# CDACHPCIE25/PPQSFLHE

Hardware: AMD Instinct MI355X
Metric: ciphertexts/sec aggregated+PRE at N=2^16, L=12 RNS limbs (higher is better)
Workload: dtype u64

## Files before the change

### ppqsflhe_amd/csrc/engine.hip

```cpp
#include "engine.hpp"
#include "comm.hpp"
#include "ntt_radix.hpp"
#include "qsum_kernels.hpp"
#include "fanout_kernels.hpp"
#include "codec_kernels.hpp"
#include "sampler_kernels.hpp"

#include <cmath>
#include <cstdio>
#include <type_traits>
#include <cstdlib>
#include <cstring>

namespace mk {


template <bool INV>
__global__ __launch_bounds__(NTT_THREADS) void k_ntt_col(NttIo io, NttTables T, const u64 *scale,
                                                         const u64 *scale_sh) {
    extern __shared__ __attribute__((aligned(16))) u64 lds[];
    const uint32_t poly = blockIdx.y / io.nslots, s = blockIdx.y % io.nslots;
    if (ntt_slot_skipped(io, poly, io.vslot0 + s)) return;
    const uint32_t id = limb_id_of(io.vslot0 + s, io.nl, T.L);
    const LimbConst lc = T.limb[id];
// ... 361 lines not shown

static int fast_row(uint32_t log_r2, uint32_t rows);

static dim3 ew_grid(uint32_t n, uint32_t slots, uint32_t items) {
    return dim3((n / 2 + EW_THREADS - 1) / EW_THREADS, slots, items);
}

static std::string hip_runtime_diagnosis() {
    std::vector<std::string> paths;
    if (FILE *f = std::fopen("/proc/self/maps", "r")) {
        char line[4096];
        while (std::fgets(line, sizeof line, f)) {
            const char *p = std::strstr(line, "libamdhip64");
            if (!p) continue;
            const char *start = std::strchr(line, '/');
            if (!start) continue;
            std::string path(start);
            while (!path.empty() && (path.back() == '\n' || path.back() == ' ')) path.pop_back();
            bool seen = false;
            for (const std::string &q : paths) seen = seen || q == path;
            if (!seen) paths.push_back(path);
        }
        std::fclose(f);
    }
    if (paths.size() < 2) return "";
    std::string msg = "; this process carries " + std::to_string(paths.size()) + " HIP runtimes (";
    for (size_t i = 0; i < paths.size(); ++i) msg += (i ? ", " : "") + paths[i];
    return msg + "): the one initialised second sees no device -- load the library that owns the device first (import torch "
                 "before libmkckks_hip.so, or link both against the same libamdhip64)";
}

static bool env_flag(const char *name, bool dflt) {
    const char *e = std::getenv(name);
    return e ? std::atoi(e) != 0 : dflt;
}
Knobs Knobs::from_env() {
    Knobs k;
    if (const char *e = std::getenv("MKCKKS_CHUNK")) {
        const int v = std::atoi(e);
        if (v >= 1 && v <= 64) k.chunk = (uint32_t)v;
    }
    if (const char *e = std::getenv("MKCKKS_QSUM_GROUP")) {
        const int v = std::atoi(e);
        if (v >= 1 && v <= 64) k.qsum_group = (uint32_t)v;
    }
    if (const char *e = std::getenv("MKCKKS_FANOUT_GROUP")) {
        const int v = std::atoi(e);
        if (v >= 1 && v <= 64) k.fanout_group = (uint32_t)v;
    }
    k.cu_affine = env_flag("MKCKKS_CU_AFFINE", k.cu_affine);
    k.generic_ntt = env_flag("MKCKKS_GENERIC_NTT", k.generic_ntt);
    k.no_pm = env_flag("MKCKKS_NO_PM", k.no_pm);
    k.no_fp64 = env_flag("MKCKKS_NO_FP64", k.no_fp64);
    return k;
}

Engine::Engine(const ParamSet &ps, int device) : ps_(ps), device_(device), knobs_(Knobs::from_env()) {
    if (device_ < 0) return;
    int count = 0;
    if (hipGetDeviceCount(&count) != hipSuccess || count <= device_)
        throw NoDevice("no HIP device " + std::to_string(device_) + " (found " + std::to_string(count) + ")" +
                       hip_runtime_diagnosis());
    MK_HIP(hipSetDevice(device_));
    const uint32_t D = ps_.D, n = ps_.n;
    tabs_.log_n = ps_.log_n;
    tabs_.log_r1 = (ps_.log_n % 2 == 0) ? ((ps_.log_n / 2) & ~1u) : ps_.log_n / 2;
    tabs_.log_r2 = ps_.log_n - tabs_.log_r1;
    if (knobs_.generic_ntt) { tabs_.log_r1 = ps_.log_n / 2; tabs_.log_r2 = ps_.log_n - tabs_.log_r1; }
    const bool radix_both = fast_log_h(tabs_.log_r1, 1u << tabs_.log_r2) && fast_row(tabs_.log_r2, 1u << tabs_.log_r1);
    const bool fp_ok = radix_both && !knobs_.no_fp64;
    tabs_.has_fp = 0;
    fp_of_.assign(D, 0);
    for (uint32_t i = 0; i < D; ++i) {
        ps_.limb[i].fp = (fp_ok && ps_.moduli[i] < (5ull << 48)) ? 1u : 0u;
        fp_of_[i] = (uint8_t)ps_.limb[i].fp;
        tabs_.has_fp |= ps_.limb[i].fp;
    }
    bool all_pm = radix_both && !knobs_.no_pm;
    for (uint32_t i = 0; i < D; ++i)
        if (!ps_.limb[i].fp && !pm_eligible(ps_.moduli[i])) all_pm = false;
    tabs_.int_pm = all_pm ? 1u : 0u;
    for (uint32_t i = 0; i < D; ++i) {
        const bool pm = all_pm && !ps_.limb[i].fp;
        ps_.limb[i].pm = pm ? 1u : 0u;
        ps_.limb[i].pm_c = pm ? (uint32_t)(((u64)1 << ps_.limb[i].k) - ps_.moduli[i]) : 0u;
    }
    tabs_.h_fp_of = fp_of_.data();
    tabs_.cu_affine = knobs_.cu_affine ? 1u : 0u;
    tabs_.stamps = nullptr;
    if (MK_STAMP && env_flag("MKCKKS_STAMPS", false)) {
        MK_HIP(hipMalloc(&d_stamps_, (size_t)STAMP_REGIONS * STAMP_REGION * sizeof(unsigned long long)));
        MK_HIP(hipMemset(d_stamps_, 0, (size_t)STAMP_REGIONS * STAMP_REGION * sizeof(unsigned long long)));
        tabs_.stamps = d_stamps_;
    }
    MK_HIP(hipMalloc(&d_limb_, D * sizeof(LimbConst)));
    MK_HIP(hipMemcpy(d_limb_, ps_.limb.data(), D * sizeof(LimbConst), hipMemcpyHostToDevice));
    const size_t tbytes = (size_t)D * n * sizeof(u64);
    MK_HIP(hipMalloc(&d_tw_, tbytes));
    MK_HIP(hipMalloc(&d_tw_sh_, tbytes));
    MK_HIP(hipMalloc(&d_itw_, tbytes));
    MK_HIP(hipMalloc(&d_itw_sh_, tbytes));
    std::vector<u64> w, wsh;
    auto as_fp = [&](uint32_t i) {
        const long double q = (long double)ps_.moduli[i];
        for (uint32_t k = 0; k < n; ++k) {
            const double wd = (double)w[k], wq = (double)((long double)w[k] / q);
            std::memcpy(&w[k], &wd, 8);
            std::memcpy(&wsh[k], &wq, 8);
        }
    };
    auto as_pm = [&](uint32_t i) {
        for (uint32_t k = 0; k < n; ++k) {
            wsh[k] = pm_tw_companion(w[k], ps_.limb[i]);
            w[k] = pm_tw(w[k], ps_.limb[i]);
        }
    };
    for (uint32_t i = 0; i < D; ++i) {
        ps_.twiddles(i, false, w, wsh);
        if (ps_.limb[i].fp) as_fp(i);
        if (ps_.limb[i].pm) as_pm(i);
        MK_HIP(hipMemcpy(d_tw_ + (size_t)i * n, w.data(), n * sizeof(u64), hipMemcpyHostToDevice));
        MK_HIP(hipMemcpy(d_tw_sh_ + (size_t)i * n, wsh.data(), n * sizeof(u64), hipMemcpyHostToDevice));
        ps_.twiddles(i, true, w, wsh);
        if (ps_.limb[i].fp) as_fp(i);
        if (ps_.limb[i].pm) as_pm(i);
        MK_HIP(hipMemcpy(d_itw_ + (size_t)i * n, w.data(), n * sizeof(u64), hipMemcpyHostToDevice));
        MK_HIP(hipMemcpy(d_itw_sh_ + (size_t)i * n, wsh.data(), n * sizeof(u64), hipMemcpyHostToDevice));
    }
    {
        const uint32_t slots = n / 2, M = 2 * n;
        std::vector<uint32_t> rot(slots);
        uint64_t pw = 1;
        for (uint32_t j = 0; j < slots; ++j) { rot[j] = (uint32_t)pw; pw = pw * 5 % M; }
        std::vector<double2> ksi(M + 1);
        const double pi = std::acos(-1.0);
        for (uint32_t k = 0; k <= M; ++k) {
            const double ang = 2.0 * pi * (double)k / (double)M;
            ksi[k] = double2{std::cos(ang), std::sin(ang)};
        }
        MK_HIP(hipMalloc(&d_rot_, slots * sizeof(uint32_t)));
        MK_HIP(hipMalloc(&d_ksi_, (M + 1) * sizeof(double2)));
// ... 375 lines not shown
                [&](hipStream_t s) { k_ntt_row3<INV, AR_FP><<<dim3((r1 / 4) * itemsf), NTT_THREADS, 0, s>>>(iof, T, tail); });
            break;
        case 4:
            launch_two_classes(ln, items != 0, itemsf != 0,
                [&](hipStream_t s) { with_int_arith(T, [&](auto ar) {
                    k_ntt_row_r<4, INV, decltype(ar)::value>
                        <<<dim3((r1 / 16) * items), NTT_THREADS, 0, s>>>(io, T, tail);
                }); },
                [&](hipStream_t s) { k_ntt_row_r<4, INV, AR_FP><<<dim3((r1 / 16) * itemsf), NTT_THREADS, 0, s>>>(iof, T, tail); });
            break;
        case 3:
            launch_two_classes(ln, items != 0, itemsf != 0,
                [&](hipStream_t s) { with_int_arith(T, [&](auto ar) {
                    k_ntt_row_r<3, INV, decltype(ar)::value>
                        <<<dim3((r1 / 32) * items), NTT_THREADS, 0, s>>>(io, T, tail);
                }); },
                [&](hipStream_t s) { k_ntt_row_r<3, INV, AR_FP><<<dim3((r1 / 32) * itemsf), NTT_THREADS, 0, s>>>(iof, T, tail); });
            break;
        case 2:
            launch_two_classes(ln, items != 0, itemsf != 0,
                [&](hipStream_t s) { with_int_arith(T, [&](auto ar) {
                    k_ntt_row_r<2, INV, decltype(ar)::value>
                        <<<dim3((r1 / 64) * items), NTT_THREADS, 0, s>>>(io, T, tail);
                }); },
                [&](hipStream_t s) { k_ntt_row_r<2, INV, AR_FP><<<dim3((r1 / 64) * itemsf), NTT_THREADS, 0, s>>>(iof, T, tail); });
            break;
        default: {
            if (tail.enabled) throw std::logic_error("fused tail needs the radix row kernel");
            const uint32_t tile = n < (uint32_t)NTT_TILE ? n : (uint32_t)NTT_TILE;
            k_ntt_row<INV><<<dim3(n / tile, n_polys * io0.nslots), NTT_THREADS, (size_t)tile * sizeof(u64), ln.main>>>(io0, T);
        }
    }
}

static void ntt_passes(NttIo io, const NttTables &T, uint32_t n_polys, bool inverse, const u64 *scale,
                       const u64 *scale_sh, const Lanes &s, int pack = 0) {
    if (n_polys == 0 || io.nslots == 0) return;
    NttIo second = io;
    second.in_group = 0;
    second.in = io.out;
    second.in_stride = io.out_stride;
    second.in_slot0 = io.out_slot0;
    const TailArgs none{};
    if (!inverse) {
        launch_col<false>(io, T, n_polys, nullptr, nullptr, s);
        launch_row<false>(second, T, n_polys, none, s);
    } else {
        launch_row<true>(io, T, n_polys, none, s);
        launch_col<true>(second, T, n_polys, scale, scale_sh, s, pack);
    }
    MK_HIP(hipGetLastError());
}

template <int LOG_H, int N_IN, int SRCMODE>
static void launch_conv_col_n(const ConvIo &io, const ConvIo &iof, const dim3 &grid, const dim3 &gridf, const NttTables &T,
                              const DevConv &cv, const Lanes &ln) {
    if constexpr (LOG_H >= 3) {
        const uint32_t per = grid.x / (io.nsel ? io.nsel : 1), perf = gridf.x / (iof.nsel ? iof.nsel : 1);
        if (io.nsel) with_int_arith(T, [&](auto ar) {
            k_conv_col2<LOG_H, N_IN, decltype(ar)::value, DevConv, SRCMODE>
                <<<dim3(per * ((io.nsel + 1) / 2)), NTT_THREADS, 0, ln.main>>>(io, T, cv);
        });
        if (iof.nsel)
            k_conv_col2<LOG_H, N_IN, AR_FP, DevConv, SRCMODE><<<dim3(perf * ((iof.nsel + 1) / 2)), NTT_THREADS, 0, ln.main>>>(iof, T, cv);
    } else {
        launch_two_classes(ln, io.nsel != 0, iof.nsel != 0,
            [&](hipStream_t s) { with_int_arith(T, [&](auto ar) {
                k_conv_col<LOG_H, N_IN, decltype(ar)::value, DevConv, SRCMODE>
                    <<<grid, NTT_THREADS, 0, s>>>(io, T, cv);
            }); },
            [&](hipStream_t s) { k_conv_col<LOG_H, N_IN, AR_FP, DevConv, SRCMODE><<<gridf, NTT_THREADS, 0, s>>>(iof, T, cv); });
    }
}
template <int LOG_H, int N_IN>
static void launch_conv_col_m(const ConvIo &io, const ConvIo &iof, const dim3 &grid, const dim3 &gridf, const NttTables &T,
                              const DevConv &cv, const Lanes &ln, int srcmode) {
    if constexpr (N_IN <= 4 && LOG_H >= 3) {
        if (srcmode == 1) return launch_conv_col_n<LOG_H, N_IN, 1>(io, iof, grid, gridf, T, cv, ln);
        if (srcmode == 2) return launch_conv_col_n<LOG_H, N_IN, (N_IN > 1 ? 2 : 0)>(io, iof, grid, gridf, T, cv, ln);
    }
    if (srcmode != 0) throw std::logic_error("double conversion sources: unsupported shape");
    launch_conv_col_n<LOG_H, N_IN, 0>(io, iof, grid, gridf, T, cv, ln);
}
template <int LOG_H>
static void launch_conv_col_h(const ConvIo &io0, const NttTables &T, const DevConv &cv, const Lanes &ln, int srcmode,
                              unsigned classes) {
    const uint32_t tiles = (1u << T.log_r2) / (256u >> LOG_H);
    ConvIo io = io0, iof = io0;
    io.target_mask = iof.target_mask = 0;
    for (uint32_t j = 0; j < cv.n_out; ++j) {
        const bool fp = T.h_fp_of[cv.dst_id[j]] != 0;
        if (fp && (classes & 2)) iof.target_mask |= 1ull << j;
        if (!fp && (classes & 1)) io.target_mask |= 1ull << j;
    }
    io.nsel = (uint32_t)__builtin_popcountll(io.target_mask);
    iof.nsel = (uint32_t)__builtin_popcountll(iof.target_mask);
    const dim3 grid(io.items * tiles * io.nsel), gridf(io.items * tiles * iof.nsel);
    switch (cv.n_in) {
        case 1: launch_conv_col_m<LOG_H, 1>(io, iof, grid, gridf, T, cv, ln, srcmode); break;
        case 2: launch_conv_col_m<LOG_H, 2>(io, iof, grid, gridf, T, cv, ln, srcmode); break;
        case 3: launch_conv_col_m<LOG_H, 3>(io, iof, grid, gridf, T, cv, ln, srcmode); break;
        case 4: launch_conv_col_m<LOG_H, 4>(io, iof, grid, gridf, T, cv, ln, srcmode); break;
        case 5: launch_conv_col_m<LOG_H, 5>(io, iof, grid, gridf, T, cv, ln, srcmode); break;
        case 6: launch_conv_col_m<LOG_H, 6>(io, iof, grid, gridf, T, cv, ln, srcmode); break;
        case 7: launch_conv_col_m<LOG_H, 7>(io, iof, grid, gridf, T, cv, ln, srcmode); break;
        case 8: launch_conv_col_m<LOG_H, 8>(io, iof, grid, gridf, T, cv, ln, srcmode); break;
        default: throw std::invalid_argument("base conversion fan-in unsupported");
    }
}
// ... 1118 lines not shown
```

### ppqsflhe_amd/csrc/engine.hpp

```cpp
#pragma once
#include <hip/hip_runtime.h>

#include <map>
#include <stdexcept>
#include <string>
#include <utility>
#include <vector>

#include "modarith.hpp"
#include "ntt_kernels.hpp"
#include "params.hpp"

namespace mk {

struct HipError : std::runtime_error {
    using std::runtime_error::runtime_error;
};
struct NoDevice : std::runtime_error {
    using std::runtime_error::runtime_error;
};
struct PrecisionError : std::runtime_error {
    using std::runtime_error::runtime_error;
};

#define MK_HIP(expr)                                                                              \
    do {                                                                                          \
        hipError_t _e = (expr);                                                                   \
        if (_e != hipSuccess)                                                                     \
            throw mk::HipError(std::string(#expr) + ": " + hipGetErrorString(_e) + " (" __FILE__ \
                               ":" + std::to_string(__LINE__) + ")");                             \
    } while (0)

constexpr int MAX_CONV_IN = 8;
constexpr int MAX_CONV_OUT = 40;

struct DevConv {
    uint32_t n_in, n_out;
    uint32_t src_id[MAX_CONV_IN];
    uint32_t src_slot[MAX_CONV_IN];
    uint32_t dst_id[MAX_CONV_OUT];
    uint32_t dst_slot[MAX_CONV_OUT];
    u64 hatinv[MAX_CONV_IN], hatinv_sh[MAX_CONV_IN];
    const u64 *hat;
    const double *hat_d;
    const double *hatq_d;
};

struct Lanes {
    hipStream_t main = nullptr;
};

struct Knobs {
    uint32_t chunk = 16;
    uint32_t fanout_group = 7;
    uint32_t qsum_group = 8;
    bool cu_affine = true;
    bool generic_ntt = false;
    bool no_pm = false;
    bool no_fp64 = false;
    static Knobs from_env();
};

class Engine {
public:
    explicit Engine(const ParamSet &ps, int device);
    ~Engine();
    Engine(const Engine &) = delete;
    Engine &operator=(const Engine &) = delete;

    const ParamSet &params() const { return ps_; }
    bool has_device() const { return device_ >= 0; }
    int device() const { return device_; }
    void set_stream(hipStream_t s) { stream_ = s; }
    hipStream_t stream() const { return stream_; }
    void sync();

    void *dev_alloc(size_t bytes);
    void dev_free(void *p);
    void upload(void *d, const void *h, size_t bytes);
    void download(void *h, const void *d, size_t bytes);
    void *host_alloc(size_t bytes);
    void host_free(void *p);
    uint64_t upload_async(void *d, const void *h, size_t bytes);
    uint64_t download_async(void *h, const void *d, size_t bytes);
    bool copy_done(uint64_t ticket);
    void copy_wait(uint64_t ticket);
    void fence_uploads();
    void fence_compute();
    uint64_t count_noncanonical(const u64 *ct, uint32_t n_ct, uint32_t nl);

    void ntt_forward(u64 *d, uint32_t n_polys, uint32_t nl, bool with_p);
    void ntt_inverse(u64 *d, uint32_t n_polys, uint32_t nl, bool with_p);

    void eval_add(const u64 *a, const u64 *b, u64 *out, uint32_t n_ct, uint32_t nl);
    void eval_sum(const u64 *in, u64 *out, uint32_t n_clients, uint32_t n_ct, uint32_t nl);
    void rescale(const u64 *in, u64 *out, uint32_t n_ct, uint32_t nl, const std::vector<u64> *factors);
    void mult_const(u64 *ct, uint32_t n_ct, uint32_t nl, const std::vector<u64> &factors);
    void reduce_mod(u64 *ct, uint32_t n_ct, uint32_t nl, uint32_t n_terms);
    void reduce_scatter_sum_mod(void *comm, const u64 *partial, u64 *shard, uint32_t n_ct_shard, uint32_t nl,
                                uint32_t n_ranks);

    void reencrypt_sum(const u64 *cts, const u64 *evks, u64 *out, uint32_t n_clients, uint32_t n_ct, uint32_t nl);
    void reencrypt_fanout(const u64 *ct, const u64 *evks, u64 *out, uint32_t n_keys, uint32_t n_ct, uint32_t nl);
    void compress(const u64 *in, u64 *out, uint32_t n_ct, uint32_t nl_in, uint32_t nl_out);
    void reencrypt_fanout_compact(const u64 *ct, const u64 *evks, u64 *out, uint32_t n_keys, uint32_t n_ct, uint32_t nl_in,
                                  uint32_t nl_out);
    void modup(const u64 *c1, u64 *digits, uint32_t n, uint32_t nl);
    void moddown(const u64 *in, u64 *out, uint32_t n, uint32_t nl);
    void reencrypt(const u64 *ct, const u64 *evk, u64 *out, uint32_t n_ct, uint32_t nl, bool accumulate = false);

    void keygen(const int8_t *s, const u64 *a, const int32_t *e, u64 *pk, u64 *sk);
    void rekeygen(const int8_t *s_old, const u64 *pk_new, const int8_t *u, const int32_t *e0,
// ... 85 lines not shown
```

### ppqsflhe_amd/csrc/ntt_kernels.hpp

```cpp
#pragma once
#include "modarith.hpp"

namespace mk {

constexpr int NTT_THREADS = 256;
constexpr int NTT_TILE = 4096;
constexpr int NTT_COLS = 16;

struct NttTables {
    const LimbConst *limb;
    const u64 *tw, *tw_sh;
    const u64 *itw, *itw_sh;
    const u64 *twb, *itwb;
    uint32_t log_n, log_r1, log_r2;
    uint32_t L;
    uint32_t has_fp;
    const unsigned char *h_fp_of;
    uint32_t int_pm;
    unsigned long long *stamps;
    uint32_t cu_affine;
};
constexpr int AR_INT = 0, AR_FP = 1, AR_PM = 2;

struct NttIo {
    const u64 *in;
    u64 *out;
    size_t in_stride, out_stride;
    uint32_t in_slot0, out_slot0;
    uint32_t vslot0;
    uint32_t nslots;
    uint32_t nl;
    uint32_t skip_nparts = 0, skip_alpha = 0;
    unsigned long long slot_mask = ~0ull;
    uint32_t nsel = 0;
    uint32_t in_group = 0;
    size_t in_gstride = 0;
};
MK_D size_t ntt_in_offset(const NttIo &io, uint32_t poly) {
    return io.in_group ? (size_t)(poly / io.in_group) * io.in_gstride + (size_t)(poly % io.in_group) * io.in_stride
                       : (size_t)poly * io.in_stride;
}

MK_D uint32_t nth_set_bit(unsigned long long mask, uint32_t n) {
    for (uint32_t i = 0; i < n; ++i) mask &= mask - 1;
    return (uint32_t)__builtin_ctzll(mask);
}

MK_D bool ntt_slot_skipped(const NttIo &io, uint32_t poly, uint32_t vslot) {
    if (!io.skip_nparts) return false;
    const uint32_t lo = (poly % io.skip_nparts) * io.skip_alpha;
    const uint32_t hi = lo + io.skip_alpha < io.nl ? lo + io.skip_alpha : io.nl;
    return vslot >= lo && vslot < hi;
}

MK_D uint32_t limb_id_of(uint32_t vslot, uint32_t nl, uint32_t L) {
    return vslot < nl ? vslot : L + (vslot - nl);
}

MK_D void ct_butterfly(u64 &x, u64 &y, u64 w, u64 wp, u64 q, u64 q2) {
    u64 u = csub(x, q2);
    u64 v = shoup_lazy(y, w, wp, q);
    x = u + v;
    y = u - v + q2;
}
MK_D void ct_butterfly_c4(u64 &x, u64 &y, u64 w, u64 wp, u64 q, u64 q2, u64 q4) {
    u64 u = csub(x, q4);
    u64 v = shoup_lazy(y, w, wp, q);
    x = u + v;
    y = u - v + q2;
}
MK_D void ct_butterfly_nc(u64 &x, u64 &y, u64 w, u64 wp, u64 q, u64 q2) {
    u64 v = shoup_lazy(y, w, wp, q);
    u64 u = x;
// ... 68 lines not shown
```

### ppqsflhe_amd/csrc/ntt_radix.hpp

```cpp
#pragma once
#include "modarith.hpp"
#include "ntt_kernels.hpp"

namespace mk {

#ifndef MK_NT8
#define MK_NT8 0
#endif
MK_D u64 ld_stream(const u64 *p) { return (MK_NT && MK_NT8) ? __builtin_nontemporal_load(p) : *p; }
MK_D ulong2 ld_stream2(const ulong2 *p) {
    if (MK_NT) {
        ulong2 v;
        v.x = __builtin_nontemporal_load(&p->x);
        v.y = __builtin_nontemporal_load(&p->y);
        return v;
    }
    return *p;
}
MK_D u64 ld_pass(const u64 *p) { return (MK_NT >= 2 && MK_NT8) ? __builtin_nontemporal_load(p) : *p; }
#ifndef MK_NT8S
#define MK_NT8S 1
#endif
MK_D void st_pass(u64 *p, u64 v) {
    if (MK_NT >= 2 && MK_NT8S) __builtin_nontemporal_store(v, p);
// ... 514 lines not shown
#pragma unroll
            for (int k = 0; k < H; ++k) {
                const u64 v = (AR == AR_FP) ? fp_to_canonical(fp_mulmod(bitsd(x[k]), bitsd(sc), bitsd(sc_sh), lc.qd), lc.qd, lc.qinv)
                                 : shoup_mul(x[k], sc, sc_sh, lc.q);
                st_pass(dst + (size_t)(j + H * k) * r2, pack30(v));
            }
        } else {
#pragma unroll
            for (int k = 0; k < H; ++k) {
                const u64 v = (AR == AR_FP) ? fp_to_canonical(fp_mulmod(bitsd(x[k]), bitsd(sc), bitsd(sc_sh), lc.qd), lc.qd, lc.qinv)
                                 : shoup_mul(x[k], sc, sc_sh, lc.q);
                st_pass(dst + (size_t)(j + H * k) * r2, v);
            }
        }
    }
}

struct ConvIo {
    const u64 *in;
    u64 *out;
    size_t in_stride, out_stride;
    uint32_t items;
    unsigned long long target_mask;
    uint32_t nsel;
};
#ifndef MK_CONV_DEPTH
#define MK_CONV_DEPTH 6
#endif
#ifndef MK_PROBE
#define MK_PROBE 0
#endif
#if MK_PROBE == 1
#define MK_PROBE_SRC(src, limb_off, row_off) (src)[(limb_off) + (size_t)j * r2 + 0 * (row_off)]
#elif MK_PROBE == 2
#define MK_PROBE_SRC(src, limb_off, row_off) ((u64)threadIdx.x * 0x9E3779B97F4A7C15ull + (limb_off) + (row_off))
#else
#define MK_PROBE_SRC(src, limb_off, row_off) (src)[(limb_off) + (row_off)]
#endif

MK_D void split30_d(u64 dbl_bits, uint32_t &lo, uint32_t &hi) {
    const u64 b = dbits(bitsd(dbl_bits) + 4503599627370496.0) & 0xFFFFFFFFFFFFFull;
    lo = (uint32_t)b & 0x3FFFFFFFu;
    hi = (uint32_t)(b >> 30);
}
template <int SRCMODE>
MK_D constexpr bool src_is_double(int i) {
    return SRCMODE == 1 || (SRCMODE == 2 && i > 0);
}
template <int N_IN>
struct ConvConst {
    uint32_t h0[N_IN], h1[N_IN];
    double hd[N_IN], hq[N_IN];
};
template <int N_IN, int AR, int SRCMODE, typename CONV>
MK_D void conv_consts(const CONV &cv, uint32_t jt, ConvConst<N_IN> &k) {
#pragma unroll
    for (int i = 0; i < N_IN; ++i) {
        if ((AR == AR_FP) && src_is_double<SRCMODE>(i)) {
            k.hd[i] = cv.hat_d[i * cv.n_out + jt];
            k.hq[i] = cv.hatq_d[i * cv.n_out + jt];
        } else {
            split30(cv.hat[i * cv.n_out + jt], k.h0[i], k.h1[i]);
        }
    }
}
template <int N_IN, int SRCMODE>
MK_D void conv_split_sources(const u64 (&p)[N_IN], uint32_t (&a0)[N_IN], uint32_t (&a1)[N_IN]) {
#pragma unroll
    for (int i = 0; i < N_IN; ++i) {
        if (src_is_double<SRCMODE>(i)) {
            split30_d(p[i], a0[i], a1[i]);
        } else {
            a0[i] = (uint32_t)p[i];
            a1[i] = (uint32_t)(p[i] >> 32);
        }
    }
}
template <int N_IN, int AR, int SRCMODE>
MK_D u64 conv_output(const u64 (&p)[N_IN], const uint32_t (&a0)[N_IN], const uint32_t (&a1)[N_IN], const ConvConst<N_IN> &k,
                     const LimbConst &lc) {
    if ((AR == AR_FP) && SRCMODE != 0) {
        double acc = 0.0;
        if (SRCMODE == 2) {
            Cols ia{0, 0, 0};
#pragma unroll
            for (int i = 0; i < N_IN; ++i)
                if (!src_is_double<SRCMODE>(i)) mac_cols(ia, (uint32_t)p[i], (uint32_t)(p[i] >> 32), k.h0[i], k.h1[i]);
            acc = (double)reduce_cols_lazy(ia, lc);
        }
#pragma unroll
        for (int i = 0; i < N_IN; ++i)
            if (src_is_double<SRCMODE>(i)) acc += fp_mulmod(bitsd(p[i]), k.hd[i], k.hq[i], lc.qd);
        return dbits(fp_reduce(acc, lc.qd, lc.qinv));
    }
    Cols acc{0, 0, 0};
#pragma unroll
    for (int i = 0; i < N_IN; ++i) mac_cols(acc, a0[i], a1[i], k.h0[i], k.h1[i]);
    const u64 v = AR == AR_PM ? pm_reduce_cols(acc, pm_consts(lc)) : reduce_cols_lazy(acc, lc);
    return AR == AR_FP ? dbits(fp_reduce((double)v, lc.qd, lc.qinv)) : v;
}

template <int LOG_H, int N_IN, int AR, typename CONV, int SRCMODE = 0>
__global__ __launch_bounds__(NTT_THREADS, 4) void k_conv_col(ConvIo io, NttTables T, CONV cv) {
    using TL = ColTile<LOG_H>;
    constexpr int H = TL::H, S = TL::S;
    static_assert(SRCMODE == 0 || N_IN <= 4, "double sources: at most 4 per digit");
    __shared__ u64 lds[TL::WORDS + ColTwB<LOG_H>::WORDS];
    const uint32_t n = 1u << T.log_n, r2 = 1u << T.log_r2, tiles = r2 / S;
    const uint32_t groups = io.items * tiles;
    uint32_t grp, jt;
    group_member(blockIdx.x, groups, io.nsel, T.cu_affine, grp, jt);
    jt = nth_set_bit(io.target_mask, jt);
    uint32_t item, tile;
    conv_item_tile(grp, groups, io.items, tiles, item, tile);
    const uint32_t id = cv.dst_id[jt];
// ... 7 lines not shown
    stm.mark<0>();
    if constexpr (N_IN <= 4) {
        ConvConst<N_IN> kc;
        conv_consts<N_IN, AR, SRCMODE>(cv, jt, kc);
        constexpr int DEPTH = MK_CONV_DEPTH < H ? MK_CONV_DEPTH : H;
        u64 ring[DEPTH][N_IN];
#pragma unroll
        for (int k = 0; k < DEPTH; ++k)
#pragma unroll
            for (int i = 0; i < N_IN; ++i) ring[k][i] = MK_PROBE_SRC(src, (size_t)cv.src_slot[i] * n, (size_t)(j + H * k) * r2);
#pragma unroll
        for (int k = 0; k < H; ++k) {
            u64 p[N_IN];
#pragma unroll
            for (int i = 0; i < N_IN; ++i) p[i] = ring[k % DEPTH][i];
            if (k + DEPTH < H) {
#pragma unroll
                for (int i = 0; i < N_IN; ++i)
                    ring[k % DEPTH][i] = MK_PROBE_SRC(src, (size_t)cv.src_slot[i] * n, (size_t)(j + H * (k + DEPTH)) * r2);
            }
            uint32_t a0[N_IN], a1[N_IN];
            if (!((AR == AR_FP) && SRCMODE != 0)) conv_split_sources<N_IN, SRCMODE>(p, a0, a1);
            x[k] = conv_output<N_IN, AR, SRCMODE>(p, a0, a1, kc, lc);
            asm volatile("" : "+v"(x[k]));
            __builtin_amdgcn_sched_barrier(0);
        }
    } else {
        uint32_t h0[N_IN], h1[N_IN];
#pragma unroll
        for (int i = 0; i < N_IN; ++i) split30(cv.hat[i * cv.n_out + jt], h0[i], h1[i]);
#pragma unroll
        for (int k = 0; k < H; ++k) {
            Cols4 acc{0, 0, 0, 0};
#pragma unroll
            for (int i = 0; i < N_IN; ++i) {
                const u64 p = src[(size_t)cv.src_slot[i] * n + (size_t)(j + H * k) * r2];
                mac_cols4(acc, (uint32_t)p, (uint32_t)(p >> 32), h0[i], h1[i]);
            }
            x[k] = reduce_cols4(acc, lc);
            if (AR == AR_FP) x[k] = dbits(fp_reduce((double)x[k], lc.qd, lc.qinv));
            asm volatile("" : "+v"(x[k]));
            __builtin_amdgcn_sched_barrier(0);
        }
    }
    stm.mark<1>();
    col_forward_finish<LOG_H, AR>(x, lds, T.tw + (size_t)id * n, T.tw_sh + (size_t)id * n, lc, j, c, dst, r2, &stm);
    if (AR == AR_FP) stm.flush<0>(T.stamps, true);
    else stm.flush<1>(T.stamps, true);
}

#ifndef MK_CONV2_DEPTH
#define MK_CONV2_DEPTH 4
#endif
template <int LOG_H, int N_IN, int AR, typename CONV, int SRCMODE = 0>
__global__ __launch_bounds__(NTT_THREADS, 3) void k_conv_col2(ConvIo io, NttTables T, CONV cv) {
    using TL = ColTile<LOG_H>;
    constexpr int H = TL::H, S = TL::S;
    static_assert(SRCMODE == 0 || N_IN <= 4, "double sources: at most 4 per digit");
    __shared__ u64 lds[TL::WORDS + ColTwB<LOG_H>::WORDS];
    const uint32_t n = 1u << T.log_n, r2 = 1u << T.log_r2, tiles = r2 / S;
    const uint32_t groups = io.items * tiles, ntg = (io.nsel + 1) / 2;
    uint32_t grp, jg;
    group_member(blockIdx.x, groups, ntg, T.cu_affine, grp, jg);
    const bool two = jg * 2 + 1 < io.nsel;
    const uint32_t jta = nth_set_bit(io.target_mask, jg * 2), jtb = two ? nth_set_bit(io.target_mask, jg * 2 + 1) : jta;
    uint32_t item, tile;
    conv_item_tile(grp, groups, io.items, tiles, item, tile);
    const uint32_t ida = cv.dst_id[jta], idb = cv.dst_id[jtb];
    const LimbConst la = T.limb[ida], lb = T.limb[idb];
    if ((la.fp != 0) != (AR == AR_FP) || (lb.fp != 0) != (AR == AR_FP)) return;
    const int c = threadIdx.x % S, j = threadIdx.x / S;
    const u64 *src = io.in + (size_t)item * io.in_stride + tile * S + c;
    u64 xa[H], xb[H];
    if constexpr (N_IN > 4) {
        uint32_t h0a[N_IN], h1a[N_IN], h0b[N_IN], h1b[N_IN];
#pragma unroll
        for (int i = 0; i < N_IN; ++i) {
            split30(cv.hat[i * cv.n_out + jta], h0a[i], h1a[i]);
            split30(cv.hat[i * cv.n_out + jtb], h0b[i], h1b[i]);
        }
#pragma unroll
        for (int k = 0; k < H; ++k) {
            Cols4 acca{0, 0, 0, 0}, accb{0, 0, 0, 0};
#pragma unroll
            for (int i = 0; i < N_IN; ++i) {
                const u64 p = src[(size_t)cv.src_slot[i] * n + (size_t)(j + H * k) * r2];
                mac_cols4(acca, (uint32_t)p, (uint32_t)(p >> 32), h0a[i], h1a[i]);
                mac_cols4(accb, (uint32_t)p, (uint32_t)(p >> 32), h0b[i], h1b[i]);
            }
            xa[k] = reduce_cols4(acca, la);
            xb[k] = reduce_cols4(accb, lb);
            if (AR == AR_FP) {
                xa[k] = dbits(fp_reduce((double)xa[k], la.qd, la.qinv));
                xb[k] = dbits(fp_reduce((double)xb[k], lb.qd, lb.qinv));
            }
            asm volatile("" : "+v"(xa[k]), "+v"(xb[k]));
            __builtin_amdgcn_sched_barrier(0);
        }
    } else {
    ConvConst<N_IN> ka, kb;
    conv_consts<N_IN, AR, SRCMODE>(cv, jta, ka);
    conv_consts<N_IN, AR, SRCMODE>(cv, jtb, kb);
    constexpr int DEPTH = MK_CONV2_DEPTH < H ? MK_CONV2_DEPTH : H;
    u64 ring[DEPTH][N_IN];
#pragma unroll
    for (int k = 0; k < DEPTH; ++k)
#pragma unroll
        for (int i = 0; i < N_IN; ++i) ring[k][i] = src[(size_t)cv.src_slot[i] * n + (size_t)(j + H * k) * r2];
#pragma unroll
    for (int k = 0; k < H; ++k) {
        u64 p[N_IN];
#pragma unroll
        for (int i = 0; i < N_IN; ++i) p[i] = ring[k % DEPTH][i];
        if (k + DEPTH < H) {
#pragma unroll
            for (int i = 0; i < N_IN; ++i)
                ring[k % DEPTH][i] = src[(size_t)cv.src_slot[i] * n + (size_t)(j + H * (k + DEPTH)) * r2];
        }
        uint32_t a0[N_IN], a1[N_IN];
        if (!((AR == AR_FP) && SRCMODE != 0)) conv_split_sources<N_IN, SRCMODE>(p, a0, a1);
        xa[k] = conv_output<N_IN, AR, SRCMODE>(p, a0, a1, ka, la);
        xb[k] = conv_output<N_IN, AR, SRCMODE>(p, a0, a1, kb, lb);
        asm volatile("" : "+v"(xa[k]), "+v"(xb[k]));
        __builtin_amdgcn_sched_barrier(0);
    }
    }
    u64 *dst = io.out + (size_t)item * io.out_stride + (size_t)cv.dst_slot[jta] * n + tile * S + c;
    col_forward_finish<LOG_H, AR>(xa, lds, T.tw + (size_t)ida * n, T.tw_sh + (size_t)ida * n, la, j, c, dst, r2);
    if (!two) return;
    __syncthreads();
    dst = io.out + (size_t)item * io.out_stride + (size_t)cv.dst_slot[jtb] * n + tile * S + c;
    const u64 *twb = T.tw + (size_t)idb * n, *twb_sh = T.tw_sh + (size_t)idb * n;
    asm volatile("" : "+s"(twb), "+s"(twb_sh));
    col_forward_finish<LOG_H, AR>(xb, lds, twb, twb_sh, lb, j, c, dst, r2);
}

template <int LOG_H, int AR>
__global__ __launch_bounds__(NTT_THREADS, 3) void k_icol_sum(const u64 *pc, u64 *psum, NttTables T, const u64 *scale,
                                                             const u64 *scale_sh, uint32_t K, uint32_t n_clients,
                                                             size_t in_cstride) {
    using TL = ColTile<LOG_H>;
    constexpr int H = TL::H, S = TL::S;
    static_assert(AR != AR_FP, "P limbs are integer-class");
    __shared__ u64 lds[TL::WORDS + ColTwB<LOG_H>::WORDS];
    const uint32_t poly = blockIdx.y / K, k = blockIdx.y % K;
    const uint32_t id = T.L + k;
    const LimbConst lc = T.limb[id];
    const uint32_t n = 1u << T.log_n, r2 = 1u << T.log_r2;
    const int c = threadIdx.x % S, j = threadIdx.x / S;
    const size_t off = ((size_t)poly * K + k) * n + blockIdx.x * S + c;
    const u64 *itw0 = T.itw + (size_t)id * n, *itw_sh0 = T.itw_sh + (size_t)id * n;
    const u64 sc = scale[id], sc_sh = scale_sh[id];
    u64 acc[H];
#pragma unroll
    for (int kk = 0; kk < H; ++kk) acc[kk] = 0;
    ColTwB<LOG_H>::stage(lds + TL::WORDS, itw0, itw_sh0);
    wave_lds_sync();
    const u64 *strip = lds + TL::WORDS;
#pragma unroll 1
    for (uint32_t cl = 0; cl < n_clients; ++cl) {
        const u64 *src = pc + (size_t)cl * in_cstride + off;
        u64 x[H];
        uint32_t r2v = r2;
        asm volatile("" : "+s"(r2v));
#pragma unroll
        for (int kk = 0; kk < H; ++kk) x[kk] = ld_pass(src + (uint32_t)(H * j + kk) * r2v);
        radix_inverse_staged<LOG_H, AR>(x, [&](int i) { return ColTwB<LOG_H>::pair_b(strip, j, i); }, lc);
        if (cl) __syncthreads();
#pragma unroll
        for (int kk = 0; kk < H; ++kk) lds[TL::at(j, kk, c)] = x[kk];
        __syncthreads();
#pragma unroll
        for (int kk = 0; kk < H; ++kk) x[kk] = lds[TL::at(kk, j, c)];
        radix_inverse_staged<LOG_H, AR>(x, [&](int i) { return ColTwB<LOG_H>::pair_a(strip, i); }, lc);
#pragma unroll
        for (int kk = 0; kk < H; ++kk) acc[kk] += shoup_mul(x[kk], sc, sc_sh, lc.q);
    }
    u64 *dst = psum + off;
#pragma unroll
    for (int kk = 0; kk < H; ++kk) st_pass(dst + (size_t)(j + H * kk) * r2, acc[kk]);
}

template <int LOG_H, int N_IN, int AR, typename CONV>
__global__ __launch_bounds__(NTT_THREADS, 4) void k_conv_col_psum(ConvIo io, NttTables T, CONV cv) {
    using TL = ColTile<LOG_H>;
    constexpr int H = TL::H, S = TL::S;
    __shared__ u64 lds[TL::WORDS + ColTwB<LOG_H>::WORDS];
// ... 1059 lines not shown
```

Before: 31710.

## Merge int and fp basis-conversion column launches into one mixed-pair kernel

Adds a k_conv_col_mix kernel that handles integer-class and fp64-class conversion targets in a single launch. Targets are paired host-side, preferring same-class pairs and producing at most one mixed pair, and blocks are placed onto CUs with an optional two-CU grouping scheme. It also moves per-target hat constants into scalar registers via readfirstlane. The aim is to remove a separate launch, fill the GPU better, and lower VGPR pressure. The cost is extra template instantiations and branching, and the mixed pair may be unbalanced.

```diff
diff --git a/ppqsflhe_amd/csrc/engine.hip b/ppqsflhe_amd/csrc/engine.hip
--- a/ppqsflhe_amd/csrc/engine.hip
+++ b/ppqsflhe_amd/csrc/engine.hip
@@ -437,6 +437,10 @@
     k.generic_ntt = env_flag("MKCKKS_GENERIC_NTT", k.generic_ntt);
     k.no_pm = env_flag("MKCKKS_NO_PM", k.no_pm);
     k.no_fp64 = env_flag("MKCKKS_NO_FP64", k.no_fp64);
+    if (const char *e = std::getenv("MKCKKS_CONV_SPLIT")) {
+        const int v = std::atoi(e);
+        if (v >= 0 && v <= 3) k.conv_split = (uint32_t)v;
+    }
     return k;
 }
 
@@ -472,6 +476,7 @@
     }
     tabs_.h_fp_of = fp_of_.data();
     tabs_.cu_affine = knobs_.cu_affine ? 1u : 0u;
+    tabs_.conv_split = knobs_.conv_split;
     tabs_.stamps = nullptr;
     if (MK_STAMP && env_flag("MKCKKS_STAMPS", false)) {
         MK_HIP(hipMalloc(&d_stamps_, (size_t)STAMP_REGIONS * STAMP_REGION * sizeof(unsigned long long)));
@@ -953,9 +958,40 @@
     MK_HIP(hipGetLastError());
 }
 
+static ConvPairs conv_pairs(unsigned long long mask_int, unsigned long long mask_fp) {
+    static_assert(MAX_CONV_OUT <= 2 * CONV_MAX_PAIRS, "ConvPairs holds every target of a digit");
+    std::vector<uint32_t> ti, tf;
+    for (uint32_t j = 0; j < (uint32_t)MAX_CONV_OUT; ++j) {
+        if ((mask_int >> j) & 1) ti.push_back(j);
+        if ((mask_fp >> j) & 1) tf.push_back(j);
+    }
+    ConvPairs pr{};
+    size_t a = 0, b = 0;
+    while (a + 1 < tf.size() || b + 1 < ti.size()) {
+        if (a + 1 < tf.size()) { pr.pair[pr.n++] = tf[a] | (tf[a + 1] << 8); a += 2; }
+        if (b + 1 < ti.size()) { pr.pair[pr.n++] = ti[b] | (ti[b + 1] << 8); b += 2; }
+    }
+    if (a < tf.size() && b < ti.size()) pr.pair[pr.n++] = tf[a] | (ti[b] << 8);
+    else if (a < tf.size()) pr.pair[pr.n++] = tf[a] | (tf[a] << 8);
+    else if (b < ti.size()) pr.pair[pr.n++] = ti[b] | (ti[b] << 8);
+    return pr;
+}
 template <int LOG_H, int N_IN, int SRCMODE>
 static void launch_conv_col_n(const ConvIo &io, const ConvIo &iof, const dim3 &grid, const dim3 &gridf, const NttTables &T,
                               const DevConv &cv, const Lanes &ln) {
+    if constexpr (LOG_H >= 3 && N_IN <= 4 && SRCMODE != 0) {
+        if (T.conv_split != 1 && io.nsel && iof.nsel) {
+            ConvPairs pr = conv_pairs(io.target_mask, iof.target_mask);
+            const uint32_t per = grid.x / io.nsel;
+            pr.place = T.conv_split == 2 ? 1u : (T.conv_split == 0 && T.cu_affine && per % 128 == 0) ? 2u : 0u;
+            const uint32_t members = pr.place == 2 ? (pr.n + 1) / 2 * 2 : pr.n;
+            with_int_arith(T, [&](auto ar) {
+                k_conv_col_mix<LOG_H, N_IN, decltype(ar)::value, DevConv, SRCMODE>
+                    <<<dim3(per * members), NTT_THREADS, 0, ln.main>>>(io, T, cv, pr);
+            });
+            return;
+        }
+    }
     if constexpr (LOG_H >= 3) {
         const uint32_t per = grid.x / (io.nsel ? io.nsel : 1), perf = gridf.x / (iof.nsel ? iof.nsel : 1);
         if (io.nsel) with_int_arith(T, [&](auto ar) {
diff --git a/ppqsflhe_amd/csrc/engine.hpp b/ppqsflhe_amd/csrc/engine.hpp
--- a/ppqsflhe_amd/csrc/engine.hpp
+++ b/ppqsflhe_amd/csrc/engine.hpp
@@ -58,6 +58,7 @@
     bool generic_ntt = false;
     bool no_pm = false;
     bool no_fp64 = false;
+    uint32_t conv_split = 0;
     static Knobs from_env();
 };
 
diff --git a/ppqsflhe_amd/csrc/ntt_kernels.hpp b/ppqsflhe_amd/csrc/ntt_kernels.hpp
--- a/ppqsflhe_amd/csrc/ntt_kernels.hpp
+++ b/ppqsflhe_amd/csrc/ntt_kernels.hpp
@@ -19,6 +19,7 @@
     uint32_t int_pm;
     unsigned long long *stamps;
     uint32_t cu_affine;
+    uint32_t conv_split;
 };
 constexpr int AR_INT = 0, AR_FP = 1, AR_PM = 2;
 
diff --git a/ppqsflhe_amd/csrc/ntt_radix.hpp b/ppqsflhe_amd/csrc/ntt_radix.hpp
--- a/ppqsflhe_amd/csrc/ntt_radix.hpp
+++ b/ppqsflhe_amd/csrc/ntt_radix.hpp
@@ -590,15 +590,28 @@
     uint32_t h0[N_IN], h1[N_IN];
     double hd[N_IN], hq[N_IN];
 };
-template <int N_IN, int AR, int SRCMODE, typename CONV>
+MK_D double to_sgpr(double v) {
+    const u64 b = dbits(v);
+    const uint32_t lo = __builtin_amdgcn_readfirstlane((uint32_t)b), hi = __builtin_amdgcn_readfirstlane((uint32_t)(b >> 32));
+    return bitsd((u64)hi << 32 | lo);
+}
+template <int N_IN, int AR, int SRCMODE, bool TO_SGPR = false, typename CONV>
 MK_D void conv_consts(const CONV &cv, uint32_t jt, ConvConst<N_IN> &k) {
 #pragma unroll
     for (int i = 0; i < N_IN; ++i) {
         if ((AR == AR_FP) && src_is_double<SRCMODE>(i)) {
             k.hd[i] = cv.hat_d[i * cv.n_out + jt];
             k.hq[i] = cv.hatq_d[i * cv.n_out + jt];
+            if (TO_SGPR) {
+                k.hd[i] = to_sgpr(k.hd[i]);
+                k.hq[i] = to_sgpr(k.hq[i]);
+            }
         } else {
             split30(cv.hat[i * cv.n_out + jt], k.h0[i], k.h1[i]);
+            if (TO_SGPR) {
+                k.h0[i] = __builtin_amdgcn_readfirstlane(k.h0[i]);
+                k.h1[i] = __builtin_amdgcn_readfirstlane(k.h1[i]);
+            }
         }
     }
 }
@@ -712,6 +725,53 @@
 #ifndef MK_CONV2_DEPTH
 #define MK_CONV2_DEPTH 4
 #endif
+template <int LOG_H, int N_IN, int ARA, int ARB, int SRCMODE, bool TO_SGPR = false, typename CONV>
+MK_D void conv_pair_outputs(const u64 *src, const CONV &cv, uint32_t n, uint32_t r2, int j, uint32_t jta, uint32_t jtb,
+                            const LimbConst &la, const LimbConst &lb, u64 (&xa)[1 << LOG_H], u64 (&xb)[1 << LOG_H]) {
+    constexpr int H = 1 << LOG_H;
+    ConvConst<N_IN> ka, kb;
+    conv_consts<N_IN, ARA, SRCMODE, TO_SGPR>(cv, jta, ka);
+    conv_consts<N_IN, ARB, SRCMODE, TO_SGPR>(cv, jtb, kb);
+    constexpr int DEPTH = MK_CONV2_DEPTH < H ? MK_CONV2_DEPTH : H;
+    u64 ring[DEPTH][N_IN];
+#pragma unroll
+    for (int k = 0; k < DEPTH; ++k)
+#pragma unroll
+        for (int i = 0; i < N_IN; ++i) ring[k][i] = src[(size_t)cv.src_slot[i] * n + (size_t)(j + H * k) * r2];
+#pragma unroll
+    for (int k = 0; k < H; ++k) {
+        u64 p[N_IN];
+#pragma unroll
+        for (int i = 0; i < N_IN; ++i) p[i] = ring[k % DEPTH][i];
+        if (k + DEPTH < H) {
+#pragma unroll
+            for (int i = 0; i < N_IN; ++i)
+                ring[k % DEPTH][i] = src[(size_t)cv.src_slot[i] * n + (size_t)(j + H * (k + DEPTH)) * r2];
+        }
+        uint32_t a0[N_IN], a1[N_IN];
+        if (!((ARA == AR_FP) && (ARB == AR_FP) && SRCMODE != 0)) conv_split_sources<N_IN, SRCMODE>(p, a0, a1);
+        xa[k] = conv_output<N_IN, ARA, SRCMODE>(p, a0, a1, ka, la);
+        xb[k] = conv_output<N_IN, ARB, SRCMODE>(p, a0, a1, kb, lb);
+        asm volatile("" : "+v"(xa[k]), "+v"(xb[k]));
+        __builtin_amdgcn_sched_barrier(0);
+    }
+}
+template <int LOG_H, int ARA, int ARB, typename CONV>
+MK_D void conv_pair_finish(u64 (&xa)[1 << LOG_H], u64 (&xb)[1 << LOG_H], u64 *lds, const ConvIo &io, const NttTables &T,
+                           const CONV &cv, uint32_t item, uint32_t tile, uint32_t jta, uint32_t jtb, uint32_t ida,
+                           uint32_t idb, const LimbConst &la, const LimbConst &lb, bool two, int j, int c, uint32_t n,
+                           uint32_t r2) {
+    constexpr int S = ColTile<LOG_H>::S;
+    u64 *dst = io.out + (size_t)item * io.out_stride + (size_t)cv.dst_slot[jta] * n + tile * S + c;
+    col_forward_finish<LOG_H, ARA>(xa, lds, T.tw + (size_t)ida * n, T.tw_sh + (size_t)ida * n, la, j, c, dst, r2);
+    if (!two) return;
+    __syncthreads();
+    dst = io.out + (size_t)item * io.out_stride + (size_t)cv.dst_slot[jtb] * n + tile * S + c;
+    const u64 *twb = T.tw + (size_t)idb * n, *twb_sh = T.tw_sh + (size_t)idb * n;
+    asm volatile("" : "+s"(twb), "+s"(twb_sh));
+    col_forward_finish<LOG_H, ARB>(xb, lds, twb, twb_sh, lb, j, c, dst, r2);
+}
+
 template <int LOG_H, int N_IN, int AR, typename CONV, int SRCMODE = 0>
 __global__ __launch_bounds__(NTT_THREADS, 3) void k_conv_col2(ConvIo io, NttTables T, CONV cv) {
     using TL = ColTile<LOG_H>;
@@ -758,41 +818,57 @@
             __builtin_amdgcn_sched_barrier(0);
         }
     } else {
-    ConvConst<N_IN> ka, kb;
-    conv_consts<N_IN, AR, SRCMODE>(cv, jta, ka);
-    conv_consts<N_IN, AR, SRCMODE>(cv, jtb, kb);
-    constexpr int DEPTH = MK_CONV2_DEPTH < H ? MK_CONV2_DEPTH : H;
-    u64 ring[DEPTH][N_IN];
-#pragma unroll
-    for (int k = 0; k < DEPTH; ++k)
-#pragma unroll
-        for (int i = 0; i < N_IN; ++i) ring[k][i] = src[(size_t)cv.src_slot[i] * n + (size_t)(j + H * k) * r2];
-#pragma unroll
-    for (int k = 0; k < H; ++k) {
-        u64 p[N_IN];
-#pragma unroll
-        for (int i = 0; i < N_IN; ++i) p[i] = ring[k % DEPTH][i];
-        if (k + DEPTH < H) {
-#pragma unroll
-            for (int i = 0; i < N_IN; ++i)
-                ring[k % DEPTH][i] = src[(size_t)cv.src_slot[i] * n + (size_t)(j + H * (k + DEPTH)) * r2];
-        }
-        uint32_t a0[N_IN], a1[N_IN];
-        if (!((AR == AR_FP) && SRCMODE != 0)) conv_split_sources<N_IN, SRCMODE>(p, a0, a1);
-        xa[k] = conv_output<N_IN, AR, SRCMODE>(p, a0, a1, ka, la);
-        xb[k] = conv_output<N_IN, AR, SRCMODE>(p, a0, a1, kb, lb);
-        asm volatile("" : "+v"(xa[k]), "+v"(xb[k]));
-        __builtin_amdgcn_sched_barrier(0);
-    }
-    }
-    u64 *dst = io.out + (size_t)item * io.out_stride + (size_t)cv.dst_slot[jta] * n + tile * S + c;
-    col_forward_finish<LOG_H, AR>(xa, lds, T.tw + (size_t)ida * n, T.tw_sh + (size_t)ida * n, la, j, c, dst, r2);
-    if (!two) return;
-    __syncthreads();
-    dst = io.out + (size_t)item * io.out_stride + (size_t)cv.dst_slot[jtb] * n + tile * S + c;
-    const u64 *twb = T.tw + (size_t)idb * n, *twb_sh = T.tw_sh + (size_t)idb * n;
-    asm volatile("" : "+s"(twb), "+s"(twb_sh));
-    col_forward_finish<LOG_H, AR>(xb, lds, twb, twb_sh, lb, j, c, dst, r2);
+        conv_pair_outputs<LOG_H, N_IN, AR, AR, SRCMODE>(src, cv, n, r2, j, jta, jtb, la, lb, xa, xb);
+    }
+    conv_pair_finish<LOG_H, AR, AR>(xa, xb, lds, io, T, cv, item, tile, jta, jtb, ida, idb, la, lb, two, j, c, n, r2);
+}
+
+constexpr int CONV_MAX_PAIRS = 20;
+struct ConvPairs {
+    uint32_t n;
+    uint32_t place;
+    uint32_t pair[CONV_MAX_PAIRS];
+};
+MK_D bool group_member_2cu(uint32_t b, uint32_t members, uint32_t &grp, uint32_t &mem) {
+    const uint32_t half = (members + 1) / 2, xcd = b % 8, qidx = b / 8;
+    const uint32_t per = 32 * half, blk = qidx / per, r = qidx % per, c = r % 32;
+    grp = (blk * 16 + c / 2) * 8 + xcd;
+    mem = (c % 2) * half + r / 32;
+    return mem < members;
+}
+template <int LOG_H, int N_IN, int AR_I, typename CONV, int SRCMODE>
+__global__ __launch_bounds__(NTT_THREADS, 3) void k_conv_col_mix(ConvIo io, NttTables T, CONV cv, ConvPairs pr) {
+    using TL = ColTile<LOG_H>;
+    constexpr int H = TL::H, S = TL::S;
+    static_assert(N_IN <= 4 && SRCMODE != 0, "one-launch conversion: double sources, at most 4 per digit");
+    __shared__ u64 lds[TL::WORDS + ColTwB<LOG_H>::WORDS];
+    const uint32_t n = 1u << T.log_n, r2 = 1u << T.log_r2, tiles = r2 / S;
+    const uint32_t groups = io.items * tiles;
+    uint32_t grp, jg;
+    if (pr.place == 2) {
+        if (!group_member_2cu(blockIdx.x, pr.n, grp, jg)) return;
+    } else {
+        group_member(blockIdx.x, groups, pr.n, T.cu_affine && !pr.place, grp, jg);
+    }
+    const uint32_t pw = pr.pair[jg], jta = pw & 0xFFu, jtb = pw >> 8;
+    const bool two = jta != jtb;
+    uint32_t item, tile;
+    conv_item_tile(grp, groups, io.items, tiles, item, tile);
+    const uint32_t ida = cv.dst_id[jta], idb = cv.dst_id[jtb];
+    const LimbConst la = T.limb[ida], lb = T.limb[idb];
+    const int c = threadIdx.x % S, j = threadIdx.x / S;
+    const u64 *src = io.in + (size_t)item * io.in_stride + tile * S + c;
+    u64 xa[H], xb[H];
+    if (la.fp && lb.fp) {
+        conv_pair_outputs<LOG_H, N_IN, AR_FP, AR_FP, SRCMODE, true>(src, cv, n, r2, j, jta, jtb, la, lb, xa, xb);
+        conv_pair_finish<LOG_H, AR_FP, AR_FP>(xa, xb, lds, io, T, cv, item, tile, jta, jtb, ida, idb, la, lb, two, j, c, n, r2);
+    } else if (!la.fp && !lb.fp) {
+        conv_pair_outputs<LOG_H, N_IN, AR_I, AR_I, SRCMODE, true>(src, cv, n, r2, j, jta, jtb, la, lb, xa, xb);
+        conv_pair_finish<LOG_H, AR_I, AR_I>(xa, xb, lds, io, T, cv, item, tile, jta, jtb, ida, idb, la, lb, two, j, c, n, r2);
+    } else if (la.fp) {
+        conv_pair_outputs<LOG_H, N_IN, AR_FP, AR_I, SRCMODE, true>(src, cv, n, r2, j, jta, jtb, la, lb, xa, xb);
+        conv_pair_finish<LOG_H, AR_FP, AR_I>(xa, xb, lds, io, T, cv, item, tile, jta, jtb, ida, idb, la, lb, two, j, c, n, r2);
+    }
 }
 
 template <int LOG_H, int AR>
```

After: 31990, median of 6. No clear change (+0.9%).
